# zyhbili/Dual-Space-NeRF

Measured on AMD Instinct MI355X. Metric: rendered rays/sec (64 samples/ray), 512x512 frame, higher is better.
Workload: dtype split-f16x3 (3 x v_mfma_f32_32x32x16_f16 on hi/lo fp16 operand halves, f32 accumulate: f32-equivalent accuracy - parity bars of the tests: 1e-4 absolute on RGB / acc / weights against the reference; sigma 1e-4 absolute where |sigma| <= 100 and 4e-6 RELATIVE to max|sigma| above (this checkpoint: |sig

## Files before the change

### dual-space-nerf_amd/csrc/dsn_field16.hip

```cpp
#include "dsn_common.h"
#include "dsn_kernels.h"

typedef float f32x16 __attribute__((ext_vector_type(16)));
typedef _Float16 half8 __attribute__((ext_vector_type(8)));
#define MFMA16(a, b, c) __builtin_amdgcn_mfma_f32_32x32x16_f16((a), (b), (c), 0, 0, 0)

#if !defined(DSN_EXPERIMENTS) && (defined(F16_ABL) || defined(F16_SABL) || defined(F16_TIMING) || defined(F16_TRAIN_ABL))
#error "F16_ABL / F16_SABL / F16_TIMING are experiment switches (wrong results / debug counters): build with -DDSN_EXPERIMENTS"
#endif
#ifndef F16_SINCOS_OCML
#define F16_SINCOS_OCML 0
#endif
#ifndef F16_FENCE
#define F16_FENCE 0
#endif
#ifndef F16_SGB
#define F16_SGB 1
#endif
#ifndef F16_SGB_VALU
#define F16_SGB_VALU 2
#endif
#ifndef F16_SGB_DS
#define F16_SGB_DS 1
#endif
#ifndef F16_MIX
#define F16_MIX 1
#endif
#ifndef F16_PIPE_LATE
#define F16_PIPE_LATE 1
#endif
#ifndef F16_ABL
#define F16_ABL 0
#endif
#ifndef F16_NEXT_POINT
#define F16_NEXT_POINT 1
#endif
#ifndef F16_DMA_SPREAD
#define F16_DMA_SPREAD 1
#endif
#ifndef F16_BIAS_AHEAD
#define F16_BIAS_AHEAD 1
#endif
#ifndef F16_TIMING
#define F16_TIMING 0
#endif
#ifndef F16_PREFETCH
#define F16_PREFETCH 1
#endif

#define F16_THREADS 256
#if defined(DSN_EXPERIMENTS) && defined(F16_TRAIN_ABL) && (F16_TRAIN_ABL & 32)
#define F16_ST_M(m) (1024 * (m))
#else
#define F16_ST_M(m) (32 * (m))
#endif
#define F16_CHUNK 8
#define F16_RING_SLOTS (2 * F16_CHUNK)
#define F16_NCHUNK (DSN_STREAM_BLOCKS / F16_CHUNK)
#define F16_RANGE 65000.0f
#define F16_RANGE_SCALED 32768.0f
#define F16_GSCALE 0.015625f
#define F16_GUNSCALE 64.0f

#if F16_TIMING
__device__ unsigned long long g_f16_timing[16];
#define F16_STAMP(i) do { if (MODE == F16_FWD) { asm volatile("s_waitcnt vmcnt(0) lgkmcnt(0)" ::: "memory"); tstamp[i] = __builtin_readcyclecounter(); rstamp[i] = wall_clock64(); } } while (0)
extern "C" __attribute__((visibility("default"))) int dsn_debug_timing(unsigned long long* out16, int reset) {
    if (out16 && hipMemcpyFromSymbol(out16, HIP_SYMBOL(g_f16_timing), sizeof(unsigned long long) * 16) != hipSuccess) return 1;
    if (reset) { unsigned long long z[16] = {0}; if (hipMemcpyToSymbol(HIP_SYMBOL(g_f16_timing), z, sizeof(z)) != hipSuccess) return 1; }
    return 0;
}
#else
#define F16_STAMP(i) do { } while (0)
#endif
struct W16 {
    const char* g;
    char* ring;
    unsigned ring_off;
    int wave;
    int nchunk = F16_NCHUNK;
    bool spread = F16_DMA_SPREAD != 0;
    half8 h0, l0, h1, l1;
};

#ifndef F16_POS_OFFS
#define F16_POS_OFFS 0
#endif
__device__ __forceinline__ void w16_stage(const W16& w, int c) {
    const char* src = w.g + (size_t)c * 32768;
    const unsigned dst = w.ring_off + (c & 1) * 32768 + w.wave * 8192 + 4096;
#if F16_POS_OFFS
    asm volatile("s_mov_b32 m0, %1\n\ts_nop 0\n\t"
                 "global_load_lds_dwordx4 %0, off\n\tglobal_load_lds_dwordx4 %0, off offset:1024\n\t"
                 "global_load_lds_dwordx4 %0, off offset:2048\n\tglobal_load_lds_dwordx4 %0, off offset:3072"
                 : : "v"(src - 4096), "s"(dst - 4096) : "memory", "m0");
    asm volatile("s_mov_b32 m0, %1\n\ts_nop 0\n\t"
                 "global_load_lds_dwordx4 %0, off\n\tglobal_load_lds_dwordx4 %0, off offset:1024\n\t"
                 "global_load_lds_dwordx4 %0, off offset:2048\n\tglobal_load_lds_dwordx4 %0, off offset:3072"
                 : : "v"(src), "s"(dst) : "memory", "m0");
    return;
#endif
    asm volatile("s_mov_b32 m0, %1\n\ts_nop 0\n\t"
                 "global_load_lds_dwordx4 %0, off offset:-4096\n\tglobal_load_lds_dwordx4 %0, off offset:-3072\n\t"
                 "global_load_lds_dwordx4 %0, off offset:-2048\n\tglobal_load_lds_dwordx4 %0, off offset:-1024\n\t"
                 "global_load_lds_dwordx4 %0, off\n\tglobal_load_lds_dwordx4 %0, off offset:1024\n\t"
                 "global_load_lds_dwordx4 %0, off offset:2048\n\tglobal_load_lds_dwordx4 %0, off offset:3072"
                 : : "v"(src), "s"(dst) : "memory", "m0");
}
template <int I>
__device__ __forceinline__ void w16_stage_part(const W16& w, int c) {
    const char* src = w.g + (size_t)c * 32768;
    const unsigned dst = w.ring_off + (c & 1) * 32768 + w.wave * 8192 + 4096;
// ... 141 lines not shown
__device__ __forceinline__ f32x16 unscale16(const f32x16& m, const f32x16& c) {
    f32x16 v;
#pragma unroll
    for (int r = 0; r < 16; ++r) v[r] = (m[r] + c[r]) * F16_FWD_INV;
    return v;
}
__device__ __forceinline__ f32x16 fold16(const f32x16& m, const f32x16& c) {
    f32x16 v;
#pragma unroll
    for (int r = 0; r < 16; ++r) v[r] = fmaf(c[r], DSN_LO_INV, m[r]);
    return v;
}
__device__ __forceinline__ uint32_t dsn_push_sign(uint32_t word, float v) {
    return __builtin_amdgcn_alignbit(word, __float_as_uint(v), 31);
}
__device__ __forceinline__ uint32_t dsn_active_word(uint32_t signs) { return ~signs & 0xffffu; }
#ifndef F16_KEEP_ASM
#define F16_KEEP_ASM 1
#endif
__device__ __forceinline__ float dsn_keep_active(float v, uint32_t word, int r) {
#if F16_KEEP_ASM
    uint32_t m;
    asm("v_bfe_i32 %0, %1, %2, 1" : "=v"(m) : "v"(word), "s"(15 - r));
    return __uint_as_float(__float_as_uint(v) & m);
#else
    return __uint_as_float(__float_as_uint(v) & (uint32_t)__builtin_amdgcn_sbfe((int)word, 15 - r, 1));
#endif
}
__device__ __forceinline__ uint32_t relu_bits16(f32x16& a) {
    uint32_t s = 0;
#pragma unroll
    for (int r = 0; r < 16; ++r) {
        s = dsn_push_sign(s, a[r]);
        a[r] = fmaxf(a[r], 0.0f);
    }
    return dsn_active_word(s);
}
__device__ __forceinline__ void mask16(f32x16& a, uint32_t m) {
#pragma unroll
    for (int r = 0; r < 16; ++r) a[r] = dsn_keep_active(a[r], m, r);
}

__device__ __forceinline__ void track16(float& ovf, const f32x16& v) {
#pragma unroll
    for (int r = 0; r < 16; r += 2) asm("v_max3_f32 %0, %0, |%1|, |%2|" : "+v"(ovf) : "v"(v[r]), "v"(v[r + 1]));
}
__device__ __forceinline__ float dsn_nan_flag() { return __uint_as_float(0x7fc00000u); }

#if defined(DSN_EXPERIMENTS) && defined(F16_TRAIN_ABL) && (F16_TRAIN_ABL & 256)
__device__ __forceinline__ void store16_lines_emul(float* st, const float (&o)[16]) {
    const int lane = threadIdx.x & 63;
    const unsigned long long me = (unsigned long long)(uintptr_t)st;
#pragma unroll
    for (int j = 0; j < 4; ++j) {
        const int src = 8 * j + (lane >> 3);
        const unsigned lo = __shfl((unsigned)me, src), hi = __shfl((unsigned)(me >> 32), src);
        float* pj = reinterpret_cast<float*>((uintptr_t)(((unsigned long long)hi << 32) | lo));
        if (pj) *reinterpret_cast<float4*>(pj + 4 * (lane & 7)) = make_float4(o[4 * j], o[4 * j + 1], o[4 * j + 2], o[4 * j + 3]);
    }
}
#endif
template <bool FWD, bool ST = false, bool HEAD = false>
__device__ __forceinline__ void epi_slice(const f32x16& pM, const f32x16& pC, int kb, uint32_t mword, uint32_t& bits,
                                          half8 (&yh)[2], half8 (&yl)[2], float& ovf, float* st = nullptr, float stscale = 1.0f,
                                          const float* wd = nullptr, float* sg = nullptr) {
#if F16_ABL & 16
    {
        asm volatile("" : : "a"(pM[2 * kb]), "a"(pM[2 * kb + 1]), "a"(pC[2 * kb]), "a"(pC[2 * kb + 1]));
        if (kb == 0) { yh[0] = yh[1]; yl[0] = yl[1]; }
        return;
    }
#endif
    float vv[2];
#pragma unroll
    for (int e = 0; e < 2; ++e) {
        const int r = 2 * kb + e;
#if F16_ABL & 32
        asm volatile("" : : "v"(pC[r]));
        float v = FWD ? pM[r] * F16_FWD_INV : pM[r];
#else
        float v = FWD ? (pM[r] + pC[r]) * F16_FWD_INV : fmaf(pC[r], DSN_LO_INV, pM[r]);
#endif
        if (FWD) {
            bits = dsn_push_sign(bits, v);
            v = fmaxf(v, 0.0f);
        } else {
            v = dsn_keep_active(v, mword, r);
        }
        vv[e] = v;
        if (HEAD) *sg = fmaf(wd[8 * (r >> 2) + (r & 3)], v, *sg);
#if !F16_MIX
        const _Float16 hi = (_Float16)v;
        const float res = fmaf((float)hi, -1.0f, v);
        yh[r >> 3][r & 7] = hi;
        yl[r >> 3][r & 7] = FWD ? (_Float16)res : (_Float16)(res * DSN_LO_SCALE);
#endif
    }
#if F16_MIX
    {
        const int r = 2 * kb;
        uint32_t H, L;
        asm("v_cvt_pk_f16_f32 %0, %1, %2" : "=v"(H) : "v"(vv[0]), "v"(vv[1]));
        if (FWD) {
            asm("v_fma_mixlo_f16 %0, %1, -1.0, %2 op_sel_hi:[1,0,0]" : "=v"(L) : "v"(H), "v"(vv[0]));
            asm("v_fma_mixhi_f16 %0, %1, -1.0, %2 op_sel:[1,0,0] op_sel_hi:[1,0,0]" : "+v"(L) : "v"(H), "v"(vv[1]));
        } else {
            const float k = -DSN_LO_SCALE;
            const float s0 = vv[0] * DSN_LO_SCALE, s1 = vv[1] * DSN_LO_SCALE;
            asm("v_fma_mixlo_f16 %0, %1, %2, %3 op_sel_hi:[1,0,0]" : "=v"(L) : "v"(H), "s"(k), "v"(s0));
            asm("v_fma_mixhi_f16 %0, %1, %2, %3 op_sel:[1,0,0] op_sel_hi:[1,0,0]" : "+v"(L) : "v"(H), "s"(k), "v"(s1));
        }
        typedef uint32_t u32x4 __attribute__((ext_vector_type(4)));
        u32x4 th = __builtin_bit_cast(u32x4, yh[r >> 3]), tl = __builtin_bit_cast(u32x4, yl[r >> 3]);
        th[(r & 7) >> 1] = H;
        tl[(r & 7) >> 1] = L;
        yh[r >> 3] = __builtin_bit_cast(half8, th);
        yl[r >> 3] = __builtin_bit_cast(half8, tl);
    }
#endif
    if (FWD) asm("v_max3_f32 %0, %0, %1, %2" : "+v"(ovf) : "v"(vv[0]), "v"(vv[1]));
    else asm("v_max3_f32 %0, %0, |%1|, |%2|" : "+v"(ovf) : "v"(vv[0]), "v"(vv[1]));
#if defined(DSN_EXPERIMENTS) && defined(F16_TRAIN_ABL) && (F16_TRAIN_ABL & 256)
    if (ST && kb == 7) {
        float o[16];
#pragma unroll
        for (int r = 0; r < 16; ++r) {
            float v = FWD ? (pM[r] + pC[r]) * F16_FWD_INV : fmaf(pC[r], DSN_LO_INV, pM[r]);
            v = FWD ? fmaxf(v, 0.0f) : dsn_keep_active(v, mword, r);
            o[r] = v * stscale;
        }
        store16_lines_emul(st, o);
        return;
    }
#endif
    if (ST && kb == 7 && st) {
#pragma unroll
        for (int q = 0; q < 4; ++q) {
            float o[4];
#pragma unroll
            for (int e = 0; e < 4; ++e) {
                const int r = 4 * q + e;
                float v = FWD ? (pM[r] + pC[r]) * F16_FWD_INV : fmaf(pC[r], DSN_LO_INV, pM[r]);
                v = FWD ? fmaxf(v, 0.0f) : dsn_keep_active(v, mword, r);
                o[e] = v * stscale;
            }
            *reinterpret_cast<float4*>(st + 8 * q) = make_float4(o[0], o[1], o[2], o[3]);
        }
    }
}
#ifndef F16_NT_STORE
#define F16_NT_STORE 0
#endif
typedef float f32x4 __attribute__((ext_vector_type(4)));
__device__ __forceinline__ void store16(float* st, const f32x16& v, float stscale) {
#if defined(DSN_EXPERIMENTS) && defined(F16_TRAIN_ABL) && (F16_TRAIN_ABL & 4)
    {
        const int lane = threadIdx.x & 63, hf = lane >> 5, i = lane & 3;
        const unsigned long long me = (unsigned long long)(uintptr_t)st;
#pragma unroll
        for (int j = 0; j < 4; ++j) {
            const int src = (lane & ~3) | j;
            const unsigned lo = __shfl((unsigned)me, src), hi = __shfl((unsigned)(me >> 32), src);
            float* pj = reinterpret_cast<float*>((uintptr_t)(((unsigned long long)hi << 32) | lo));
            if (pj) *reinterpret_cast<float4*>(pj - 4 * hf + 16 * hf + 4 * i) =
                make_float4(v[4 * j] * stscale, v[4 * j + 1] * stscale, v[4 * j + 2] * stscale, v[4 * j + 3] * stscale);
        }
        return;
// ... 22 lines not shown

template <bool ST = false, bool EXTRA = false, bool HEAD = false>
__device__ __forceinline__ void layer16_fwd(W16& w, int& blk, int lane, const float* __restrict__ bias,
                                            const half8 (&xh)[8][2], const half8 (&xl)[8][2], half8 (&yh)[8][2],
                                            half8 (&yl)[8][2], uint32_t (&mk)[4], float& ovf, float* st = nullptr,
                                            const half8 (*s_pe)[F16_THREADS] = nullptr, const float* wden = nullptr, float* sg = nullptr) {
    const int half = lane >> 5;
    const int tid = threadIdx.x;
    f32x16 pM = zero16(), pC = zero16();
#if F16_BIAS_AHEAD
    f32x16 bnext = rows16(bias, 0, half);
#endif
#pragma unroll
    for (int m = 0; m < 8; ++m) {
#if F16_BIAS_AHEAD
        f32x16 aM = bnext, aC = zero16();
        if (m + 1 < 8) bnext = rows16(bias, m + 1, half);
#else
        f32x16 aM = rows16(bias, m, half), aC = zero16();
#endif
        uint32_t bits = 0;
        if (m == 0) dense16<8, false>(w, blk, lane, xh, xl, aM, aC);
        else dense16<8, false>(w, blk, lane, xh, xl, aM, aC, [&](int kb) {
            epi_slice<true, ST, HEAD>(pM, pC, kb, 0u, bits, yh[m - 1], yl[m - 1], ovf, (ST && st) ? st + F16_ST_M(m - 1) : nullptr, 1.0f,
                                      HEAD ? wden + 32 * (m - 1) + 4 * half : nullptr, sg); });
        if (EXTRA) {
            half8 qh[2][2], ql[2][2];
            qh[0][0] = s_pe[0][tid]; qh[0][1] = s_pe[1][tid]; qh[1][0] = s_pe[2][tid]; qh[1][1] = s_pe[3][tid];
            ql[0][0] = s_pe[4][tid]; ql[0][1] = s_pe[5][tid]; ql[1][0] = s_pe[6][tid]; ql[1][1] = s_pe[7][tid];
            dense16<2, false>(w, blk, lane, qh, ql, aM, aC);
        }
        if (m > 0) { if ((m - 1) & 1) mk[(m - 1) >> 1] |= dsn_active_word(bits) << 16; else mk[(m - 1) >> 1] = dsn_active_word(bits); }
        pM = aM; pC = aC;
    }
    {
        uint32_t bits = 0;
#pragma unroll
        for (int kb = 0; kb < 8; ++kb)
            epi_slice<true, ST, HEAD>(pM, pC, kb, 0u, bits, yh[7], yl[7], ovf, (ST && st) ? st + F16_ST_M(7) : nullptr, 1.0f,
                                      HEAD ? wden + 32 * 7 + 4 * half : nullptr, sg);
        mk[3] |= dsn_active_word(bits) << 16;
    }
}
template <bool ST = false>
__device__ __forceinline__ void layer16_bwd(W16& w, int& blk, int lane, const half8 (&xh)[8][2],
                                            const half8 (&xl)[8][2], half8 (&yh)[8][2], half8 (&yl)[8][2],
                                            const uint32_t (&mk)[4], float& ovf, float* st = nullptr, float stscale = F16_GUNSCALE) {
    f32x16 pM = zero16(), pC = zero16();
    uint32_t dummy = 0;
#pragma unroll
    for (int m = 0; m < 8; ++m) {
        f32x16 aM = zero16(), aC = zero16();
        const uint32_t mw = m > 0 ? ((mk[(m - 1) >> 1] >> (16 * ((m - 1) & 1))) & 0xffffu) : 0u;
        if (m == 0) dense16<8, true>(w, blk, lane, xh, xl, aM, aC);
        else dense16<8, true>(w, blk, lane, xh, xl, aM, aC, [&](int kb) { epi_slice<false, ST>(pM, pC, kb, mw, dummy, yh[m - 1], yl[m - 1], ovf, (ST && st) ? st + F16_ST_M(m - 1) : nullptr, stscale); });
        pM = aM; pC = aC;
    }
    const uint32_t mw = (mk[3] >> 16) & 0xffffu;
#pragma unroll
    for (int kb = 0; kb < 8; ++kb) epi_slice<false, ST>(pM, pC, kb, mw, dummy, yh[7], yl[7], ovf, (ST && st) ? st + F16_ST_M(7) : nullptr, stscale);
}

#define F16_FULL 0
#define F16_FWD 1
#define F16_BWD 2
#define F16_TRAIN 3
#define F16_DEN 4
#define F16_FIRST_BWD_BLOCK (OFF_L6T / DSN_BLK)
#define F16_DEN_BLOCKS (F16_FIRST_BWD_BLOCK - 4 * 8)
static_assert(F16_DEN_BLOCKS % F16_CHUNK == 0, "the density-only kernel streams whole chunks");
template <int MODE>
__global__ void __launch_bounds__(F16_THREADS, 1)
k_field16(const float* __restrict__ packed, const DsnFrameState* __restrict__ fs, const float* __restrict__ x_c,
          int64_t N, const int32_t* __restrict__ active_list, const int32_t* __restrict__ active_count,
          float* __restrict__ sigma, float* __restrict__ essence, float* __restrict__ grad,
          uint4* __restrict__ masks, int32_t* __restrict__ pos_list, int32_t* __restrict__ pos_count,
          float* __restrict__ tr_h, float* __restrict__ tr_a, float* __restrict__ tr_rr, int64_t slot_base, int64_t rec_cap,
          const int32_t* __restrict__ sel, int32_t* __restrict__ flag_count) {
    constexpr bool ST = MODE == F16_TRAIN;
    __shared__ __attribute__((aligned(16))) char ring[F16_RING_SLOTS * 4096];
    __shared__ uint32_t s_mask[7][4][F16_THREADS];
    __shared__ __attribute__((aligned(16))) float s_vec[256 + 2304 + 8];
    __shared__ __attribute__((aligned(16))) half8 s_pe[8][F16_THREADS];
    __shared__ int s_app[8];
#ifndef F16_SHARE_SIMD
    DSN_OWN_SIMD();
#endif
    const int tid0 = threadIdx.x;
    const int lane0 = threadIdx.x & 63;
    const int wave = __builtin_amdgcn_readfirstlane(threadIdx.x >> 6);
    int64_t count = (active_list ? (int64_t)(*active_count) : N) - slot_base;
    if (MODE == F16_BWD && count > rec_cap) count = rec_cap;
    const int64_t ntiles = (count + 127) / 128;
    if ((int64_t)blockIdx.x >= ntiles) return;
    for (int i = tid0; i < 256 + 2304 + 8; i += F16_THREADS)
        s_vec[i] = i < 256 ? fs->bias0[i] : (i < 2560 ? packed[OFF_B1 + (i - 256)] : packed[OFF_SCAL + (i - 2560)]);
    for (int i = tid0; i < 256 + (OFF_WDEN - OFF_B1); i += F16_THREADS) s_vec[i] *= F16_FWD_SCALE;
    const float* const v_bias0 = s_vec;
    const float* const v_b1 = s_vec + 256;
    const float* const v_brgb1 = s_vec + 256 + (OFF_BRGB1 - OFF_B1);
    const float* const v_wden = s_vec + 256 + (OFF_WDEN - OFF_B1);
    const float* const v_wrgb3 = s_vec + 256 + (OFF_WRGB3 - OFF_B1);
    const float* const v_scal = s_vec + 2560;
    W16 w;
    w.g = reinterpret_cast<const char*>(packed + OFF16_BASE) + wave * 8192 + 4096 + lane0 * 16;
    w.ring = ring;
    w.ring_off = (unsigned)(uintptr_t)(__attribute__((address_space(3))) char*)ring;
    w.wave = wave;
    if (MODE == F16_FWD) w.nchunk = F16_FIRST_BWD_BLOCK / F16_CHUNK;
    if (MODE == F16_DEN) w.nchunk = F16_DEN_BLOCKS / F16_CHUNK;
    if (MODE == F16_TRAIN) w.spread = false;
    auto tile_point = [&](int64_t t, bool& ok, int64_t& ls) -> int64_t {
        int64_t sl = (t * 4 + wave) * 32 + (lane0 & 31);
        ok = sl < count;
        if (!ok) sl = count - 1;
        ls = sel ? (int64_t)sel[sl] : slot_base + sl;
        return active_list ? (int64_t)active_list[ls] : ls;
    };
    bool valid_n;
    int64_t lslot_n;
    int64_t pt_n = tile_point(blockIdx.x, valid_n, lslot_n);
    float xn[3] = {x_c[3 * pt_n], x_c[3 * pt_n + 1], x_c[3 * pt_n + 2]};
  for (int64_t tile = blockIdx.x; tile < ntiles; tile += gridDim.x) {
    int tid = tid0, lane = lane0;
    asm volatile("" : "+v"(tid), "+v"(lane), "+v"(w.g));
    const int half = lane >> 5;
#if F16_TIMING
    unsigned long long tstamp[6], rstamp[6];
#endif
    F16_STAMP(0);
    w16_begin_issue(w, MODE == F16_BWD ? F16_FIRST_BWD_BLOCK : 0);
#if !F16_NEXT_POINT
    if (tile != (int64_t)blockIdx.x) { pt_n = tile_point(tile, valid_n, lslot_n); xn[0] = x_c[3 * pt_n]; xn[1] = x_c[3 * pt_n + 1]; xn[2] = x_c[3 * pt_n + 2]; }
#endif
    const bool valid = valid_n;
    const int64_t lslot = lslot_n, pt = pt_n;
    const float xa[3] = {xn[0], xn[1], xn[2]};
    const bool more = F16_NEXT_POINT && MODE != F16_TRAIN && tile + gridDim.x < ntiles;
    if (more) pt_n = tile_point(tile + gridDim.x, valid_n, lslot_n);
#define NEXT_POINT() do { if (more) { xn[0] = x_c[3 * pt_n]; xn[1] = x_c[3 * pt_n + 1]; xn[2] = x_c[3 * pt_n + 2]; } } while (0)
    w16_begin_wait(w, lane, MODE == F16_BWD ? F16_FIRST_BWD_BLOCK : 0);
    int blk = MODE == F16_BWD ? F16_FIRST_BWD_BLOCK : 0;
    F16_STAMP(1);

#define MK_STORE(L, mk) { if (MODE != F16_DEN) { s_mask[L][0][tid] = mk[0]; s_mask[L][1][tid] = mk[1]; s_mask[L][2][tid] = mk[2]; s_mask[L][3][tid] = mk[3]; } }
#define MK_LOAD(L, mk) { mk[0] = s_mask[L][0][tid]; mk[1] = s_mask[L][1][tid]; mk[2] = s_mask[L][2][tid]; mk[3] = s_mask[L][3][tid]; }
    uint32_t mk[4];
    half8 ah[8][2], al[8][2], bh[8][2], bl[8][2];
    float ovf = packed[DSN_SPLIT_UNSAFE_FIELD];
    uint4* mrec = masks ? masks + ((size_t)(MODE == F16_BWD ? lslot : pt) * 2 + half) * 7 : nullptr;
    const int64_t tr_ls = N * 256;
#if defined(DSN_EXPERIMENTS) && defined(F16_TRAIN_ABL)
    const int64_t pt_st = (F16_TRAIN_ABL & 8) ? (pt & 4095) : ((F16_TRAIN_ABL & 16) ? (pt & 255) : pt);
    const int64_t sl_st = (tile * 4 + wave) * 32 + (lane & 31);
    const int64_t row_off = (F16_TRAIN_ABL & 32) ? (sl_st >> 5) * 8192 + (sl_st & 31) * 32 : pt_st * 256;
    float* const th = ST && valid && !(F16_TRAIN_ABL & 1) ? tr_h + row_off + 4 * half : nullptr;
    float* const ta = ST && valid && !(F16_TRAIN_ABL & 2) ? tr_a + row_off + 4 * half : nullptr;
#else
    float* const th = ST && valid ? tr_h + pt * 256 + 4 * half : nullptr;
    float* const ta = ST && valid ? tr_a + pt * 256 + 4 * half : nullptr;
#endif

  if (MODE != F16_BWD) {
    half8 ph[2][2], pl[2][2];
    {
        f32x16 pe[2];
#pragma unroll
        for (int t = 0; t < 30; ++t) {
            float s, c;
#if F16_SINCOS_OCML
            sincosf(xa[t % 3] * (float)(1 << (t / 3)), &s, &c);
#else
            dsn_sincos(xa[t % 3] * (float)(1 << (t / 3)), s, c);
#endif
            pe[t >> 4][t & 15] = half ? c : s;
        }
        pe[1][14] = half ? xa[1] : xa[0];
        pe[1][15] = half ? 0.0f : xa[2];
        split16<false>(pe[0], ph[0], pl[0]);
        split16<false>(pe[1], ph[1], pl[1]);
        s_pe[0][tid] = ph[0][0]; s_pe[1][tid] = ph[0][1]; s_pe[2][tid] = ph[1][0]; s_pe[3][tid] = ph[1][1];
        s_pe[4][tid] = pl[0][0]; s_pe[5][tid] = pl[0][1]; s_pe[6][tid] = pl[1][0]; s_pe[7][tid] = pl[1][1];
    }

    F16_STAMP(2);
#pragma unroll
    for (int m = 0; m < 8; ++m) {
        f32x16 aM = rows16(v_bias0, m, half), aC = zero16();
        dense16<2, false>(w, blk, lane, ph, pl, aM, aC);
        f32x16 v = unscale16(aM, aC);
        const uint32_t bits = relu_bits16(v);
        if (m & 1) mk[m >> 1] |= bits << 16; else mk[m >> 1] = bits;
        if (ST) store16(th ? th + 0 * tr_ls + F16_ST_M(m) : nullptr, v, 1.0f);
        track16(ovf, v);
        split16<false>(v, ah[m], al[m]);
    }
    MK_STORE(0, mk)
    layer16_fwd<ST>(w, blk, lane, v_b1 + 0 * 256, ah, al, bh, bl, mk, ovf, th ? th + 1 * tr_ls : nullptr); MK_STORE(1, mk)
    NEXT_POINT();
    layer16_fwd<ST>(w, blk, lane, v_b1 + 1 * 256, bh, bl, ah, al, mk, ovf, th ? th + 2 * tr_ls : nullptr); MK_STORE(2, mk)
    layer16_fwd<ST>(w, blk, lane, v_b1 + 2 * 256, ah, al, bh, bl, mk, ovf, th ? th + 3 * tr_ls : nullptr); MK_STORE(3, mk)
#if F16_PIPE_LATE
    layer16_fwd<ST, true, false>(w, blk, lane, v_b1 + 3 * 256, bh, bl, ah, al, mk, ovf, th ? th + 4 * tr_ls : nullptr, s_pe);
    MK_STORE(4, mk)
    layer16_fwd<ST>(w, blk, lane, v_b1 + 4 * 256, ah, al, bh, bl, mk, ovf, th ? th + 5 * tr_ls : nullptr); MK_STORE(5, mk)
    float sg_part = 0.0f;
    layer16_fwd<ST, false, true>(w, blk, lane, v_b1 + 5 * 256, bh, bl, ah, al, mk, ovf, th ? th + 6 * tr_ls : nullptr, nullptr, v_wden,
                                 &sg_part);
#else
#pragma unroll
    for (int m = 0; m < 8; ++m) {
        f32x16 aM = rows16(v_b1 + 3 * 256, m, half), aC = zero16();
        dense16<8, false>(w, blk, lane, bh, bl, aM, aC);
        {
            half8 qh[2][2], ql[2][2];
            qh[0][0] = s_pe[0][tid]; qh[0][1] = s_pe[1][tid]; qh[1][0] = s_pe[2][tid]; qh[1][1] = s_pe[3][tid];
            ql[0][0] = s_pe[4][tid]; ql[0][1] = s_pe[5][tid]; ql[1][0] = s_pe[6][tid]; ql[1][1] = s_pe[7][tid];
            dense16<2, false>(w, blk, lane, qh, ql, aM, aC);
        }
        f32x16 v = unscale16(aM, aC);
        const uint32_t bits = relu_bits16(v);
        if (m & 1) mk[m >> 1] |= bits << 16; else mk[m >> 1] = bits;
        if (ST) store16(th ? th + 4 * tr_ls + F16_ST_M(m) : nullptr, v, 1.0f);
        track16(ovf, v);
        split16<false>(v, ah[m], al[m]);
    }
    MK_STORE(4, mk)
    layer16_fwd<ST>(w, blk, lane, v_b1 + 4 * 256, ah, al, bh, bl, mk, ovf, th ? th + 5 * tr_ls : nullptr); MK_STORE(5, mk)
    float sg_part = 0.0f;
#pragma unroll
    for (int m = 0; m < 8; ++m) {
        f32x16 aM = rows16(v_b1 + 5 * 256, m, half), aC = zero16();
        dense16<8, false>(w, blk, lane, bh, bl, aM, aC);
        f32x16 v = unscale16(aM, aC);
        const uint32_t bits = relu_bits16(v);
        if (m & 1) mk[m >> 1] |= bits << 16; else mk[m >> 1] = bits;
        if (ST) store16(th ? th + 6 * tr_ls + F16_ST_M(m) : nullptr, v, 1.0f);
        const f32x16 wd = rows16(v_wden, m, half);
#pragma unroll
        for (int r = 0; r < 16; ++r) sg_part = fmaf(wd[r], v[r], sg_part);
        track16(ovf, v);
        split16<false>(v, ah[m], al[m]);
    }
#endif
    F16_STAMP(3);
    sg_part += __shfl_xor(sg_part, 32);
    const float sg = sg_part + v_scal[0];
    const bool flag_fwd = !(fmaxf(ovf, __shfl_xor(ovf, 32)) < F16_RANGE);
    if (valid && half == 0) sigma[pt] = flag_fwd ? dsn_nan_flag() : sg;
    if (MODE != F16_TRAIN && flag_fwd && valid && half == 0 && flag_count) atomicAdd(flag_count, 1);
    ovf = flag_fwd ? __builtin_inff() : 0.0f;
    if (MODE == F16_DEN) { __syncthreads(); continue; }
    bool write_rec = ST && valid;
    if (MODE == F16_FWD) {
        const bool pos = valid && half == 0 && (sg > 0.0f || flag_fwd);
        const unsigned long long bm = __ballot(pos);
        const int cnt = __popcll(bm);
        if (lane == 0) s_app[wave] = cnt;
        __syncthreads();
        if (tid == 0) {
            const int tot = s_app[0] + s_app[1] + s_app[2] + s_app[3];
            s_app[4] = tot ? atomicAdd(pos_count, tot) : 0;
        }
        __syncthreads();
        int base = s_app[4];
        for (int k = 0; k < wave; ++k) base += s_app[k];
        const int my = base + __popcll(bm & ((1ull << lane) - 1ull));
        if (pos) pos_list[my] = (int32_t)pt;
        const int rslot = __shfl(my, lane & 31);
        write_rec = ((bm >> (lane & 31)) & 1ull) != 0 && (int64_t)rslot < rec_cap;
        mrec = masks + ((size_t)rslot * 2 + half) * 7;
    }
    if (MODE == F16_FWD || MODE == F16_TRAIN) {
        MK_STORE(6, mk)
        if (write_rec) {
#pragma unroll
            for (int L = 0; L < 7; ++L)
                mrec[L] = make_uint4(s_mask[L][0][tid], s_mask[L][1][tid], s_mask[L][2][tid], s_mask[L][3][tid]);
        }
    }
    {
        float e0 = 0.f, e1 = 0.f, e2 = 0.f;
#pragma unroll
        for (int m = 0; m < 4; ++m) {
            f32x16 aM = rows16(v_brgb1, m, half), aC = zero16();
            dense16<8, false>(w, blk, lane, ah, al, aM, aC);
            const f32x16 v = unscale16(aM, aC);
            const f32x16 w0 = rows16(v_wrgb3 + 0 * 128, m, half);
            const f32x16 w1 = rows16(v_wrgb3 + 1 * 128, m, half);
            const f32x16 w2 = rows16(v_wrgb3 + 2 * 128, m, half);
            if (ST && valid) {
                f32x16 xr;
#pragma unroll
                for (int r = 0; r < 16; ++r) xr[r] = fmaxf(v[r], 0.0f);
                store16(tr_rr + pt * 128 + 4 * half + 32 * m, xr, 1.0f);
            }
#pragma unroll
            for (int r = 0; r < 16; ++r) {
                const float x = fmaxf(v[r], 0.0f);
                e0 = fmaf(w0[r], x, e0); e1 = fmaf(w1[r], x, e1); e2 = fmaf(w2[r], x, e2);
            }
        }
        e0 += __shfl_xor(e0, 32); e1 += __shfl_xor(e1, 32); e2 += __shfl_xor(e2, 32);
        if (valid && half == 0) {
            essence[3 * pt + 0] = e0 + v_scal[1];
            essence[3 * pt + 1] = e1 + v_scal[2];
            essence[3 * pt + 2] = e2 + v_scal[3];
        }
    }

#if F16_TIMING
    F16_STAMP(4);
    if (MODE == F16_FWD && tid == 0) {
        for (int i = 0; i < 4; ++i) { atomicAdd(&g_f16_timing[i], tstamp[i + 1] - tstamp[i]); atomicAdd(&g_f16_timing[8 + i], rstamp[i + 1] - rstamp[i]); }
        atomicAdd(&g_f16_timing[7], 1ull);
    }
#endif
    if (MODE == F16_FWD) { __syncthreads(); continue; }
  } else {
#pragma unroll
    for (int L = 0; L < 7; ++L) {
        const uint4 q = mrec[L];
        s_mask[L][0][tid] = q.x; s_mask[L][1][tid] = q.y; s_mask[L][2][tid] = q.z; s_mask[L][3][tid] = q.w;
    }
    MK_LOAD(6, mk)
  }

#pragma unroll
    for (int m = 0; m < 8; ++m) {
        f32x16 g = rows16(v_wden, m, half);
#pragma unroll
        for (int r = 0; r < 16; ++r) g[r] *= F16_GSCALE;
        mask16(g, (mk[m >> 1] >> (16 * (m & 1))) & 0xffffu);
        if (ST) store16(ta ? ta + 6 * tr_ls + F16_ST_M(m) : nullptr, g, F16_GUNSCALE);
        split16<true>(g, ah[m], al[m]);
    }
    MK_LOAD(5, mk) layer16_bwd<ST>(w, blk, lane, ah, al, bh, bl, mk, ovf, ta ? ta + 5 * tr_ls : nullptr);
    if (MODE == F16_BWD) NEXT_POINT();
    MK_LOAD(4, mk) layer16_bwd<ST>(w, blk, lane, bh, bl, ah, al, mk, ovf, ta ? ta + 4 * tr_ls : nullptr);
    MK_LOAD(3, mk)
    f32x16 dpe[2];
#pragma unroll
    for (int m = 0; m < 8; ++m) {
        f32x16 aM = zero16(), aC = zero16();
        dense16<8, true>(w, blk, lane, ah, al, aM, aC);
        f32x16 v = fold16(aM, aC);
        mask16(v, (mk[m >> 1] >> (16 * (m & 1))) & 0xffffu);
        if (ST) store16(ta ? ta + 3 * tr_ls + F16_ST_M(m) : nullptr, v, F16_GUNSCALE);
        track16(ovf, v);
        split16<true>(v, bh[m], bl[m]);
    }
#pragma unroll
    for (int b = 0; b < 2; ++b) {
        f32x16 aM = zero16(), aC = zero16();
        dense16<8, true>(w, blk, lane, ah, al, aM, aC);
        dpe[b] = fold16(aM, aC);
    }
    MK_LOAD(2, mk) layer16_bwd<ST>(w, blk, lane, bh, bl, ah, al, mk, ovf, ta ? ta + 2 * tr_ls : nullptr);
    MK_LOAD(1, mk) layer16_bwd<ST>(w, blk, lane, ah, al, bh, bl, mk, ovf, ta ? ta + 1 * tr_ls : nullptr);
    MK_LOAD(0, mk) layer16_bwd<ST>(w, blk, lane, bh, bl, ah, al, mk, ovf, ta ? ta + 0 * tr_ls : nullptr);
#pragma unroll
    for (int b = 0; b < 2; ++b) {
        f32x16 aM = zero16(), aC = zero16();
        dense16<8, true>(w, blk, lane, ah, al, aM, aC);
        const f32x16 v = fold16(aM, aC);
#pragma unroll
        for (int r = 0; r < 16; ++r) dpe[b][r] += v[r];
    }

    {
        float xb[3] = {xa[0], xa[1], xa[2]};
        asm volatile("" : "+v"(xb[0]), "+v"(xb[1]), "+v"(xb[2]));
        float g[3] = {0.f, 0.f, 0.f};
#pragma unroll
        for (int t = 0; t < 30; ++t) {
            const int j = t / 3, a = t % 3;
            float s, c;
#if F16_SINCOS_OCML
            sincosf(xb[a] * (float)(1 << j), &s, &c);
#else
            dsn_sincos(xb[a] * (float)(1 << j), s, c);
#endif
            const float d = dpe[t >> 4][t & 15];
            const float term = (d * (half ? s : c)) * (float)(1 << j);
            g[a] += half ? -term : term;
        }
        const float i30 = dpe[1][14], i31 = dpe[1][15];
        if (half) g[1] += i30; else { g[0] += i30; g[2] += i31; }
        g[0] += __shfl_xor(g[0], 32); g[1] += __shfl_xor(g[1], 32); g[2] += __shfl_xor(g[2], 32);
        if (valid && half == 0) {
            grad[3 * pt] = g[0] * F16_GUNSCALE; grad[3 * pt + 1] = g[1] * F16_GUNSCALE; grad[3 * pt + 2] = g[2] * F16_GUNSCALE;
        }
    }
    const bool flagged = !(fmaxf(ovf, __shfl_xor(ovf, 32)) < F16_RANGE_SCALED);
    if (flagged && valid && half == 0) {
        if (MODE == F16_TRAIN) { if (pos_count) atomicAdd(pos_count, 1); }
        else { sigma[pt] = dsn_nan_flag(); if (flag_count) atomicAdd(flag_count, 1); }
    }
    if (MODE == F16_TRAIN) break;
    __syncthreads();
  }
}

void dsn_launch_field16(const float* packed, const DsnFrameState* fs, const float* x_c, int64_t N,
                        const int32_t* active_list, const int32_t* active_count, float* sigma, float* essence,
                        float* grad, hipStream_t st, int32_t* flag_count) {
    int64_t blocks = (N + 127) / 128;
    if (blocks == 0) return;
    hipLaunchKernelGGL(k_field16<F16_FULL>, dim3((unsigned)std::min<int64_t>(blocks, dsn_cu_count())), dim3(F16_THREADS), 0, st, packed, fs, x_c, N,
                       active_list, active_count, sigma, essence, grad, (uint4*)nullptr, (int32_t*)nullptr,
                       (int32_t*)nullptr, (float*)nullptr, (float*)nullptr, (float*)nullptr, (int64_t)0, (int64_t)0, (const int32_t*)nullptr,
                       flag_count);
}
void dsn_launch_field16_from(const float* packed, const DsnFrameState* fs, const float* x_c, int64_t N, const int32_t* list,
                             const int32_t* count, int64_t slot_base, float* sigma, float* essence, float* grad, hipStream_t st,
                             int32_t* flag_count) {
    int64_t blocks = (N - slot_base + 127) / 128;
    if (blocks <= 0) return;
    hipLaunchKernelGGL(k_field16<F16_FULL>, dim3((unsigned)std::min<int64_t>(blocks, dsn_cu_count())), dim3(F16_THREADS), 0, st, packed, fs, x_c, N, list, count, sigma,
                       essence, grad, (uint4*)nullptr, (int32_t*)nullptr, (int32_t*)nullptr, (float*)nullptr, (float*)nullptr,
                       (float*)nullptr, slot_base, (int64_t)0, (const int32_t*)nullptr, flag_count);
}
void dsn_launch_field16_train(const float* packed, const DsnFrameState* fs, const float* x_c, int64_t N, float* sigma,
                              float* essence, float* grad, float* tr_h, float* tr_a, float* tr_rr, void* masks, hipStream_t st,
                              int32_t* range_count, const int32_t* row_list, const int32_t* row_count) {
    int64_t blocks = (N + 127) / 128;
    if (blocks == 0) return;
    hipLaunchKernelGGL(k_field16<F16_TRAIN>, dim3((unsigned)blocks), dim3(F16_THREADS), 0, st, packed, fs, x_c, N,
                       row_list, row_count, sigma, essence, grad, (uint4*)masks, (int32_t*)nullptr,
                       range_count, tr_h, tr_a, tr_rr, (int64_t)0, N, (const int32_t*)nullptr, (int32_t*)nullptr);
}
void dsn_launch_field16_fwd(const float* packed, const DsnFrameState* fs, const float* x_c, int64_t N,
                            const int32_t* active_list, const int32_t* active_count, float* sigma, float* essence,
                            void* masks, int32_t* pos_list, int32_t* pos_count, hipStream_t st, int64_t rec_cap, int32_t* flag_count) {
    int64_t blocks = (N + 127) / 128;
    if (blocks == 0) return;
    hipLaunchKernelGGL(k_field16<F16_FWD>, dim3((unsigned)std::min<int64_t>(blocks, dsn_cu_count())), dim3(F16_THREADS), 0, st, packed, fs, x_c, N,
                       active_list, active_count, sigma, essence, (float*)nullptr, (uint4*)masks, pos_list, pos_count,
                       (float*)nullptr, (float*)nullptr, (float*)nullptr, (int64_t)0, rec_cap, (const int32_t*)nullptr, flag_count);
}
void dsn_launch_field16_den(const float* packed, const DsnFrameState* fs, const float* x_c, int64_t N,
                            const int32_t* active_list, const int32_t* active_count, float* sigma, hipStream_t st,
                            int32_t* flag_count) {
    int64_t blocks = (N + 127) / 128;
    if (blocks == 0) return;
    hipLaunchKernelGGL(k_field16<F16_DEN>, dim3((unsigned)std::min<int64_t>(blocks, dsn_cu_count())), dim3(F16_THREADS), 0, st, packed, fs, x_c, N,
                       active_list, active_count, sigma, (float*)nullptr, (float*)nullptr, (uint4*)nullptr, (int32_t*)nullptr,
                       (int32_t*)nullptr, (float*)nullptr, (float*)nullptr, (float*)nullptr, (int64_t)0, (int64_t)0,
                       (const int32_t*)nullptr, flag_count);
}
void dsn_launch_field16_bwd(const float* packed, const DsnFrameState* fs, const float* x_c, int64_t N,
                            const int32_t* pos_list, const int32_t* pos_count, float* grad, const void* masks,
                            hipStream_t st, float* sigma, int64_t rec_cap, const int32_t* sel, const int32_t* sel_count,
                            int32_t* flag_count) {
    int64_t blocks = ((rec_cap < N ? rec_cap : N) + 127) / 128;
    if (blocks == 0) return;
    hipLaunchKernelGGL(k_field16<F16_BWD>, dim3((unsigned)std::min<int64_t>(blocks, dsn_cu_count())), dim3(F16_THREADS), 0, st, packed, fs, x_c, N,
                       pos_list, sel ? sel_count : pos_count, sigma, (float*)nullptr, grad, (uint4*)masks, (int32_t*)nullptr,
                       (int32_t*)nullptr, (float*)nullptr, (float*)nullptr, (float*)nullptr, (int64_t)0, rec_cap, sel, flag_count);
}

__device__ __forceinline__ void epi_slice_tan(const f32x16& pM, const f32x16& pC, int kb, uint32_t mword, half8 (&yh)[2],
                                              half8 (&yl)[2], float* st, float stscale, float& ovf, float* keep = nullptr) {
    float vv[2];
#pragma unroll
    for (int e = 0; e < 2; ++e) {
        const int r = 2 * kb + e;
        const float v = dsn_keep_active((pM[r] + pC[r]) * F16_FWD_INV, mword, r);
// ... 1309 lines not shown
```

Baseline: 29.96 million.

## Pipeline MFMA epilogues, split sincos encoding across halves, precompute backward seed table

Several independent changes land together in the fused field kernel. The layer-0, RGB-head and reverse layer-3 loops now run each layer's epilogue (convert, mask, split) inside the next layer's MFMA sequence via callbacks, so VALU work overlaps matrix work. The positional encoding and its backward pass split the 30 sincos evaluations between lane halves and exchange results with permlane32_swap, which halves the transcendental work per lane. The backward seed gradient (density weights times the scale) is pre-split into hi/lo fp16 in shared memory once per block and masked per point with bit tricks; the head sign packing also uses v_alignbit. The risks are higher register pressure from the overlapped epilogues and extra shared memory, plus correctness depending on the half-swapped encoding layout.

Measured after the change: 30.23 million, median of 6. About the same (+0.9%).

```diff
diff --git a/dual-space-nerf_amd/csrc/dsn_field16.hip b/dual-space-nerf_amd/csrc/dsn_field16.hip
--- a/dual-space-nerf_amd/csrc/dsn_field16.hip
+++ b/dual-space-nerf_amd/csrc/dsn_field16.hip
@@ -28,6 +28,24 @@
 #endif
 #ifndef F16_PIPE_LATE
 #define F16_PIPE_LATE 1
+#endif
+#ifndef F16_REV_PIPE
+#define F16_REV_PIPE 1
+#endif
+#ifndef F16_ENC_SPLIT
+#define F16_ENC_SPLIT 1
+#endif
+#ifndef F16_L0_PIPE
+#define F16_L0_PIPE 1
+#endif
+#ifndef F16_SEED_TABLE
+#define F16_SEED_TABLE 1
+#endif
+#ifndef F16_HEAD_SIGN_ASM
+#define F16_HEAD_SIGN_ASM 1
+#endif
+#ifndef F16_RGB_PIPE
+#define F16_RGB_PIPE 1
 #endif
 #ifndef F16_ABL
 #define F16_ABL 0
@@ -335,7 +353,8 @@
         float v = FWD ? (pM[r] + pC[r]) * F16_FWD_INV : fmaf(pC[r], DSN_LO_INV, pM[r]);
 #endif
         if (FWD) {
-            bits = dsn_push_sign(bits, v);
+            if (HEAD && !ST && F16_HEAD_SIGN_ASM) asm("v_alignbit_b32 %0, %0, %1, 31" : "+v"(bits) : "v"(v));
+            else bits = dsn_push_sign(bits, v);
             v = fmaxf(v, 0.0f);
         } else {
             v = dsn_keep_active(v, mword, r);
@@ -524,6 +543,7 @@
     __shared__ uint32_t s_mask[7][4][F16_THREADS];
     __shared__ __attribute__((aligned(16))) float s_vec[256 + 2304 + 8];
     __shared__ __attribute__((aligned(16))) half8 s_pe[8][F16_THREADS];
+    __shared__ __attribute__((aligned(16))) _Float16 s_seed[2][2][8][16];
     __shared__ int s_app[8];
 #ifndef F16_SHARE_SIMD
     DSN_OWN_SIMD();
@@ -538,6 +558,16 @@
     for (int i = tid0; i < 256 + 2304 + 8; i += F16_THREADS)
         s_vec[i] = i < 256 ? fs->bias0[i] : (i < 2560 ? packed[OFF_B1 + (i - 256)] : packed[OFF_SCAL + (i - 2560)]);
     for (int i = tid0; i < 256 + (OFF_WDEN - OFF_B1); i += F16_THREADS) s_vec[i] *= F16_FWD_SCALE;
+    if (F16_SEED_TABLE && (MODE == F16_FULL || MODE == F16_BWD)) {
+        static_assert(F16_THREADS == 256, "one thread per trunk feature");
+        const int f = tid0;
+        const float g = packed[OFF_WDEN + f] * F16_GSCALE;
+        const _Float16 hi = (_Float16)g;
+        const float res = fmaf((float)hi, -1.0f, g);
+        const int r = 4 * ((f >> 3) & 3) + (f & 3);
+        s_seed[0][(f >> 2) & 1][f >> 5][r] = hi;
+        s_seed[1][(f >> 2) & 1][f >> 5][r] = (_Float16)(res * DSN_LO_SCALE);
+    }
     const float* const v_bias0 = s_vec;
     const float* const v_b1 = s_vec + 256;
     const float* const v_brgb1 = s_vec + 256 + (OFF_BRGB1 - OFF_B1);
@@ -607,15 +637,29 @@
     half8 ph[2][2], pl[2][2];
     {
         f32x16 pe[2];
-#pragma unroll
-        for (int t = 0; t < 30; ++t) {
-            float s, c;
+#if F16_ENC_SPLIT && !F16_SINCOS_OCML
+        if (MODE != F16_TRAIN) {
+#pragma unroll
+            for (int t = 0; t < 15; ++t) {
+                float s, c;
+                dsn_sincos(xa[t % 3] * (half ? (float)(32 << (t / 3)) : (float)(1 << (t / 3))), s, c);
+                const auto r = __builtin_amdgcn_permlane32_swap(__float_as_uint(s), __float_as_uint(c), false, false);
+                pe[t >> 4][t & 15] = __uint_as_float(r[0]);
+                pe[(t + 15) >> 4][(t + 15) & 15] = __uint_as_float(r[1]);
+            }
+        } else
+#endif
+        {
+#pragma unroll
+            for (int t = 0; t < 30; ++t) {
+                float s, c;
 #if F16_SINCOS_OCML
-            sincosf(xa[t % 3] * (float)(1 << (t / 3)), &s, &c);
+                sincosf(xa[t % 3] * (float)(1 << (t / 3)), &s, &c);
 #else
-            dsn_sincos(xa[t % 3] * (float)(1 << (t / 3)), s, c);
-#endif
-            pe[t >> 4][t & 15] = half ? c : s;
+                dsn_sincos(xa[t % 3] * (float)(1 << (t / 3)), s, c);
+#endif
+                pe[t >> 4][t & 15] = half ? c : s;
+            }
         }
         pe[1][14] = half ? xa[1] : xa[0];
         pe[1][15] = half ? 0.0f : xa[2];
@@ -626,16 +670,35 @@
     }
 
     F16_STAMP(2);
-#pragma unroll
-    for (int m = 0; m < 8; ++m) {
-        f32x16 aM = rows16(v_bias0, m, half), aC = zero16();
-        dense16<2, false>(w, blk, lane, ph, pl, aM, aC);
-        f32x16 v = unscale16(aM, aC);
-        const uint32_t bits = relu_bits16(v);
-        if (m & 1) mk[m >> 1] |= bits << 16; else mk[m >> 1] = bits;
-        if (ST) store16(th ? th + 0 * tr_ls + F16_ST_M(m) : nullptr, v, 1.0f);
-        track16(ovf, v);
-        split16<false>(v, ah[m], al[m]);
+    if (F16_L0_PIPE && MODE != F16_TRAIN) {
+        f32x16 pM = zero16(), pC = zero16();
+#pragma unroll
+        for (int m = 0; m < 8; ++m) {
+            f32x16 aM = rows16(v_bias0, m, half), aC = zero16();
+            uint32_t bits = 0;
+            if (m == 0) dense16<2, false>(w, blk, lane, ph, pl, aM, aC);
+            else dense16<2, false>(w, blk, lane, ph, pl, aM, aC, [&](int kb) {
+#pragma unroll
+                for (int q = 0; q < 4; ++q) epi_slice<true>(pM, pC, 4 * kb + q, 0u, bits, ah[m - 1], al[m - 1], ovf); });
+            if (m > 0) { if ((m - 1) & 1) mk[(m - 1) >> 1] |= dsn_active_word(bits) << 16; else mk[(m - 1) >> 1] = dsn_active_word(bits); }
+            pM = aM; pC = aC;
+        }
+        uint32_t bits = 0;
+#pragma unroll
+        for (int kb = 0; kb < 8; ++kb) epi_slice<true>(pM, pC, kb, 0u, bits, ah[7], al[7], ovf);
+        mk[3] |= dsn_active_word(bits) << 16;
+    } else {
+#pragma unroll
+        for (int m = 0; m < 8; ++m) {
+            f32x16 aM = rows16(v_bias0, m, half), aC = zero16();
+            dense16<2, false>(w, blk, lane, ph, pl, aM, aC);
+            f32x16 v = unscale16(aM, aC);
+            const uint32_t bits = relu_bits16(v);
+            if (m & 1) mk[m >> 1] |= bits << 16; else mk[m >> 1] = bits;
+            if (ST) store16(th ? th + 0 * tr_ls + F16_ST_M(m) : nullptr, v, 1.0f);
+            track16(ovf, v);
+            split16<false>(v, ah[m], al[m]);
+        }
     }
     MK_STORE(0, mk)
     layer16_fwd<ST>(w, blk, lane, v_b1 + 0 * 256, ah, al, bh, bl, mk, ovf, th ? th + 1 * tr_ls : nullptr); MK_STORE(1, mk)
@@ -723,6 +786,27 @@
     }
     {
         float e0 = 0.f, e1 = 0.f, e2 = 0.f;
+      if (F16_RGB_PIPE && MODE != F16_TRAIN) {
+        f32x16 pM = zero16(), pC = zero16();
+        auto rgb_slice = [&](int m, int kb) {
+            const float* wq = v_wrgb3 + 32 * m + 8 * (kb >> 1) + 4 * half + 2 * (kb & 1);
+            const float2 w0 = *reinterpret_cast<const float2*>(wq), w1 = *reinterpret_cast<const float2*>(wq + 128),
+                         w2 = *reinterpret_cast<const float2*>(wq + 256);
+            const float x0 = fmaxf((pM[2 * kb] + pC[2 * kb]) * F16_FWD_INV, 0.0f);
+            const float x1 = fmaxf((pM[2 * kb + 1] + pC[2 * kb + 1]) * F16_FWD_INV, 0.0f);
+            e0 = fmaf(w0.x, x0, e0); e1 = fmaf(w1.x, x0, e1); e2 = fmaf(w2.x, x0, e2);
+            e0 = fmaf(w0.y, x1, e0); e1 = fmaf(w1.y, x1, e1); e2 = fmaf(w2.y, x1, e2);
+        };
+#pragma unroll
+        for (int m = 0; m < 4; ++m) {
+            f32x16 aM = rows16(v_brgb1, m, half), aC = zero16();
+            if (m == 0) dense16<8, false>(w, blk, lane, ah, al, aM, aC);
+            else dense16<8, false>(w, blk, lane, ah, al, aM, aC, [&](int kb) { rgb_slice(m - 1, kb); });
+            pM = aM; pC = aC;
+        }
+#pragma unroll
+        for (int kb = 0; kb < 8; ++kb) rgb_slice(3, kb);
+      } else {
 #pragma unroll
         for (int m = 0; m < 4; ++m) {
             f32x16 aM = rows16(v_brgb1, m, half), aC = zero16();
@@ -743,6 +827,7 @@
                 e0 = fmaf(w0[r], x, e0); e1 = fmaf(w1[r], x, e1); e2 = fmaf(w2[r], x, e2);
             }
         }
+      }
         e0 += __shfl_xor(e0, 32); e1 += __shfl_xor(e1, 32); e2 += __shfl_xor(e2, 32);
         if (valid && half == 0) {
             essence[3 * pt + 0] = e0 + v_scal[1];
@@ -768,35 +853,77 @@
     MK_LOAD(6, mk)
   }
 
-#pragma unroll
-    for (int m = 0; m < 8; ++m) {
-        f32x16 g = rows16(v_wden, m, half);
-#pragma unroll
-        for (int r = 0; r < 16; ++r) g[r] *= F16_GSCALE;
-        mask16(g, (mk[m >> 1] >> (16 * (m & 1))) & 0xffffu);
-        if (ST) store16(ta ? ta + 6 * tr_ls + F16_ST_M(m) : nullptr, g, F16_GUNSCALE);
-        split16<true>(g, ah[m], al[m]);
+    if (F16_SEED_TABLE && MODE != F16_TRAIN) {
+        typedef uint32_t u32x4 __attribute__((ext_vector_type(4)));
+        typedef short s16x2 __attribute__((ext_vector_type(2)));
+#pragma unroll
+        for (int m = 0; m < 8; ++m) {
+            const uint32_t word = (mk[m >> 1] >> (16 * (m & 1))) & 0xffffu;
+            const uint32_t w2 = word | (word << 17);
+            const u32x4* th = reinterpret_cast<const u32x4*>(&s_seed[0][half][m][0]);
+            const u32x4* tl = reinterpret_cast<const u32x4*>(&s_seed[1][half][m][0]);
+            u32x4 h[2] = {th[0], th[1]}, l[2] = {tl[0], tl[1]};
+#pragma unroll
+            for (int p = 0; p < 8; ++p) {
+                const uint32_t keep = __builtin_bit_cast(uint32_t, __builtin_bit_cast(s16x2, w2 << (2 * p)) >> (short)15);
+                h[p >> 2][p & 3] &= keep;
+                l[p >> 2][p & 3] &= keep;
+            }
+            ah[m][0] = __builtin_bit_cast(half8, h[0]); ah[m][1] = __builtin_bit_cast(half8, h[1]);
+            al[m][0] = __builtin_bit_cast(half8, l[0]); al[m][1] = __builtin_bit_cast(half8, l[1]);
+        }
+    } else {
+#pragma unroll
+        for (int m = 0; m < 8; ++m) {
+            f32x16 g = rows16(v_wden, m, half);
+#pragma unroll
+            for (int r = 0; r < 16; ++r) g[r] *= F16_GSCALE;
+            mask16(g, (mk[m >> 1] >> (16 * (m & 1))) & 0xffffu);
+            if (ST) store16(ta ? ta + 6 * tr_ls + F16_ST_M(m) : nullptr, g, F16_GUNSCALE);
+            split16<true>(g, ah[m], al[m]);
+        }
     }
     MK_LOAD(5, mk) layer16_bwd<ST>(w, blk, lane, ah, al, bh, bl, mk, ovf, ta ? ta + 5 * tr_ls : nullptr);
     if (MODE == F16_BWD) NEXT_POINT();
     MK_LOAD(4, mk) layer16_bwd<ST>(w, blk, lane, bh, bl, ah, al, mk, ovf, ta ? ta + 4 * tr_ls : nullptr);
     MK_LOAD(3, mk)
     f32x16 dpe[2];
-#pragma unroll
-    for (int m = 0; m < 8; ++m) {
-        f32x16 aM = zero16(), aC = zero16();
-        dense16<8, true>(w, blk, lane, ah, al, aM, aC);
-        f32x16 v = fold16(aM, aC);
-        mask16(v, (mk[m >> 1] >> (16 * (m & 1))) & 0xffffu);
-        if (ST) store16(ta ? ta + 3 * tr_ls + F16_ST_M(m) : nullptr, v, F16_GUNSCALE);
-        track16(ovf, v);
-        split16<true>(v, bh[m], bl[m]);
-    }
-#pragma unroll
-    for (int b = 0; b < 2; ++b) {
-        f32x16 aM = zero16(), aC = zero16();
-        dense16<8, true>(w, blk, lane, ah, al, aM, aC);
-        dpe[b] = fold16(aM, aC);
+    if (F16_REV_PIPE && MODE != F16_TRAIN) {
+        f32x16 pM = zero16(), pC = zero16();
+        uint32_t dummy = 0;
+#pragma unroll
+        for (int m = 0; m < 8; ++m) {
+            f32x16 aM = zero16(), aC = zero16();
+            const uint32_t mw = m > 0 ? ((mk[(m - 1) >> 1] >> (16 * ((m - 1) & 1))) & 0xffffu) : 0u;
+            if (m == 0) dense16<8, true>(w, blk, lane, ah, al, aM, aC);
+            else dense16<8, true>(w, blk, lane, ah, al, aM, aC, [&](int kb) { epi_slice<false>(pM, pC, kb, mw, dummy, bh[m - 1], bl[m - 1], ovf); });
+            pM = aM; pC = aC;
+        }
+        const uint32_t mw7 = (mk[3] >> 16) & 0xffffu;
+#pragma unroll
+        for (int b = 0; b < 2; ++b) {
+            f32x16 aM = zero16(), aC = zero16();
+            if (b == 0) dense16<8, true>(w, blk, lane, ah, al, aM, aC, [&](int kb) { epi_slice<false>(pM, pC, kb, mw7, dummy, bh[7], bl[7], ovf); });
+            else dense16<8, true>(w, blk, lane, ah, al, aM, aC);
+            dpe[b] = fold16(aM, aC);
+        }
+    } else {
+#pragma unroll
+        for (int m = 0; m < 8; ++m) {
+            f32x16 aM = zero16(), aC = zero16();
+            dense16<8, true>(w, blk, lane, ah, al, aM, aC);
+            f32x16 v = fold16(aM, aC);
+            mask16(v, (mk[m >> 1] >> (16 * (m & 1))) & 0xffffu);
+            if (ST) store16(ta ? ta + 3 * tr_ls + F16_ST_M(m) : nullptr, v, F16_GUNSCALE);
+            track16(ovf, v);
+            split16<true>(v, bh[m], bl[m]);
+        }
+#pragma unroll
+        for (int b = 0; b < 2; ++b) {
+            f32x16 aM = zero16(), aC = zero16();
+            dense16<8, true>(w, blk, lane, ah, al, aM, aC);
+            dpe[b] = fold16(aM, aC);
+        }
     }
     MK_LOAD(2, mk) layer16_bwd<ST>(w, blk, lane, bh, bl, ah, al, mk, ovf, ta ? ta + 2 * tr_ls : nullptr);
     MK_LOAD(1, mk) layer16_bwd<ST>(w, blk, lane, ah, al, bh, bl, mk, ovf, ta ? ta + 1 * tr_ls : nullptr);
@@ -814,18 +941,40 @@
         float xb[3] = {xa[0], xa[1], xa[2]};
         asm volatile("" : "+v"(xb[0]), "+v"(xb[1]), "+v"(xb[2]));
         float g[3] = {0.f, 0.f, 0.f};
-#pragma unroll
-        for (int t = 0; t < 30; ++t) {
-            const int j = t / 3, a = t % 3;
-            float s, c;
+#if F16_ENC_SPLIT && !F16_SINCOS_OCML
+        if (MODE != F16_TRAIN) {
+            float dsc[30];
+#pragma unroll
+            for (int t = 0; t < 15; ++t) {
+                float s, c;
+                dsn_sincos(xb[t % 3] * (half ? (float)(32 << (t / 3)) : (float)(1 << (t / 3))), s, c);
+                const auto r = __builtin_amdgcn_permlane32_swap(__float_as_uint(c), __float_as_uint(s), false, false);
+                dsc[t] = __uint_as_float(r[0]);
+                dsc[t + 15] = __uint_as_float(r[1]);
+            }
+#pragma unroll
+            for (int t = 0; t < 30; ++t) {
+                const int j = t / 3, a = t % 3;
+                const float d = dpe[t >> 4][t & 15];
+                const float term = (d * dsc[t]) * (float)(1 << j);
+                g[a] += half ? -term : term;
+            }
+        } else
+#endif
+        {
+#pragma unroll
+            for (int t = 0; t < 30; ++t) {
+                const int j = t / 3, a = t % 3;
+                float s, c;
 #if F16_SINCOS_OCML
-            sincosf(xb[a] * (float)(1 << j), &s, &c);
+                sincosf(xb[a] * (float)(1 << j), &s, &c);
 #else
-            dsn_sincos(xb[a] * (float)(1 << j), s, c);
-#endif
-            const float d = dpe[t >> 4][t & 15];
-            const float term = (d * (half ? s : c)) * (float)(1 << j);
-            g[a] += half ? -term : term;
+                dsn_sincos(xb[a] * (float)(1 << j), s, c);
+#endif
+                const float d = dpe[t >> 4][t & 15];
+                const float term = (d * (half ? s : c)) * (float)(1 << j);
+                g[a] += half ? -term : term;
+            }
         }
         const float i30 = dpe[1][14], i31 = dpe[1][15];
         if (half) g[1] += i30; else { g[0] += i30; g[2] += i31; }
```
